# gutiKristian/VolumeRendering

Hardware: AMD Instinct MI355X
Metric: Gsamples/s (higher is better)
Workload: dtype f32

## Files before the change

volumerendering_amd/csrc/vr_p2.h:

```cpp
#pragma once
#include "vr_pw.h"

namespace VR_KNS {
using namespace vr;

#ifndef VR_P2_JUMP_MAX
#define VR_P2_JUMP_MAX 1024
#endif
constexpr int kP2JumpMax = VR_P2_JUMP_MAX;
#ifndef VR_P2_EXIT
#define VR_P2_EXIT 1
#endif
constexpr bool kP2Exit = VR_P2_EXIT != 0;
constexpr int kP2Threads = 768;
constexpr int kP2ThreadsUnlit = 1024;


struct P2Lds {
    unsigned off_x, off_y, off_z;
    int mx, my, mz;
    unsigned win_last;
    unsigned win_slabs;
    unsigned win_slots;
};

__device__ __forceinline__ uint2 lds_pair(unsigned byte_off)
{
    return *reinterpret_cast<const uint2*>(reinterpret_cast<const char*>(vr_lds_tf) + byte_off);
}

__device__ __forceinline__ void p2_fill_tables(const DevVolume& v, const P2Lds& L)
{
    char* lds = reinterpret_cast<char*>(vr_lds_tf);
    for (int e = (int)threadIdx.x; e <= v.nx; e += (int)blockDim.x) {
        const unsigned i0 = (unsigned)max(e - 1, 0), i1 = (unsigned)min(e, v.nx - 1);
        *reinterpret_cast<uint2*>(lds + L.off_x + (unsigned)e * 8u) =
            make_uint2((i0 >> kVbS) * kVbN + (i0 & kVbM), (i1 >> kVbS) * kVbN + (i1 & kVbM));
    }
    for (int e = (int)threadIdx.x; e <= v.ny; e += (int)blockDim.x) {
        const unsigned j0 = (unsigned)max(e - 1, 0), j1 = (unsigned)min(e, v.ny - 1);
        *reinterpret_cast<uint2*>(lds + L.off_y + (unsigned)e * 8u) =
            make_uint2((j0 >> kVbS) * v.brick_row + ((j0 & kVbM) << kVbS), (j1 >> kVbS) * v.brick_row + ((j1 & kVbM) << kVbS));
    }
    for (int e = (int)threadIdx.x; e <= v.nz; e += (int)blockDim.x) {
        const unsigned k0 = (unsigned)max(e - 1, 0), k1 = (unsigned)min(e, v.nz - 1);
        *reinterpret_cast<uint2*>(lds + L.off_z + (unsigned)e * 8u) =
            make_uint2((k0 >> kVbS) * v.brick_slab + ((k0 & kVbM) << (2u * kVbS)), (k1 >> kVbS) * v.brick_slab + ((k1 & kVbM) << (2u * kVbS)));
    }
}

struct P2Win {
    unsigned long long ptr;
    unsigned records;
    unsigned base;
};

template <int V>
__device__ __forceinline__ void p2_set_window(P2Win& win, const DevVolume& vol, unsigned first_slot, unsigned n_slots)
{
    const char* b = (V == V_BASIC) ? vol.a_base + (size_t)first_slot * 4u : reinterpret_cast<const char*>(vol.data) + (size_t)first_slot * 16u;
    win.ptr = (unsigned long long)reinterpret_cast<size_t>(b);
    win.records = n_slots;
    win.base = first_slot;
}
template <int V>
__device__ __forceinline__ __amdgpu_buffer_rsrc_t p2_descriptor(const P2Win& win)
{
    const unsigned lo = (unsigned)__builtin_amdgcn_readfirstlane((int)(unsigned)win.ptr), hi = (unsigned)__builtin_amdgcn_readfirstlane((int)(unsigned)(win.ptr >> 32));
    void* p = reinterpret_cast<void*>((size_t)(((unsigned long long)hi << 32) | lo));
    return __builtin_amdgcn_make_buffer_rsrc(p, V == V_BASIC ? 4 : 16, __builtin_amdgcn_readfirstlane((int)win.records), 0x00020000);
}
template <int V>
constexpr unsigned p2_window_slots() { return V == V_BASIC ? 0x3fffffffu : 0x0fffffffu; }

struct P2Addr {
    uint2 ex, ey, ez;
    float fx, fy, fz;
    int tz;
};
__device__ __forceinline__ P2Addr p2_address(const DevVolume& vol, const P2Lds& L, f3 q)
{
    P2Addr a;
    const float x = mad(q.x, (float)vol.nx, -0.5f), y = mad(q.y, (float)vol.ny, -0.5f), z = mad(q.z, (float)vol.nz, -0.5f);
    const float x0 = floorf(x), y0 = floorf(y), z0 = floorf(z);
    a.fx = x - x0;
    a.fy = y - y0;
    a.fz = z - z0;
    const int tx = min(max((int)x0, -1), L.mx), ty = min(max((int)y0, -1), L.my);
    a.tz = min(max((int)z0, -1), L.mz);
    a.ex = lds_pair(L.off_x + ((unsigned)(tx + 1) << 3));
    a.ey = lds_pair(L.off_y + ((unsigned)(ty + 1) << 3));
    a.ez = lds_pair(L.off_z + ((unsigned)(a.tz + 1) << 3));
    return a;
}
template <int V, bool MASKED, bool WIN, typename T>
__device__ __forceinline__ void p2_issue(const MarchParams& P0, const DevVolume& vol, const P2Lds& L, P2Win& win, int& n_in_w, const P2Addr& a, T (&X)[8],
                                         float& fx, float& fy, float& fz, unsigned long long keep, bool need, unsigned& dbyte, float& mrec)
{
    fx = a.fx;
    fy = a.fy;
    fz = a.fz;
    const uint2 ex = a.ex, ey = a.ey, ez = a.ez;
    const int tz = a.tz;
    unsigned az0 = ez.x, az1 = ez.y;
    if constexpr (WIN) {
        az0 -= win.base;
        az1 -= win.base;
        unsigned chk = need ? az0 : 0u;
        asm volatile("" : "+v"(chk));
        const unsigned long long out = vr_ballot(chk > L.win_last);
        if (out != 0) {
            const int kb = __builtin_amdgcn_readlane(max(tz, 0) >> kVbS, (int)__builtin_ctzll(out));
            const int span = (int)L.win_slabs - 2;
            const unsigned first = (unsigned)max(0, kb - span / 2) * vol.brick_slab, total = vol.brick_slab * (((unsigned)vol.nz + kVbM) >> kVbS);
            p2_set_window<V>(win, vol, first, min(total - first, L.win_slots));
            az0 = ez.x - win.base;
            az1 = ez.y - win.base;
            unsigned chk2 = need ? az0 : 0u;
            asm volatile("" : "+v"(chk2));
            if (vr_ballot(chk2 > L.win_last) != 0) n_in_w = 0;
        }
    }
    const unsigned r00 = ey.x + az0, r10 = ey.y + az0, r01 = ey.x + az1, r11 = ey.y + az1;
    unsigned o[8] = {r00 + ex.x, r00 + ex.y, r10 + ex.x, r10 + ex.y, r01 + ex.x, r01 + ex.y, r11 + ex.x, r11 + ex.y};
    if constexpr (MASKED) {
        static_assert(kBrickShift == (int)kVbS, "the skipping's bricks are the layout's bricks");
        const unsigned bid = (WIN ? o[0] + win.base : o[0]) >> (3u * kVbS);
        dbyte = dist_at(P0, (int)bid);
        if constexpr (V == V_VOLUME_MASK) mrec = brick_record(P0, (int)bid).y;
    }
    const __amdgpu_buffer_rsrc_t rsrc = p2_descriptor<V>(win);
    unsigned long long exec_saved = 0;
    if constexpr (MASKED) {
        asm volatile("" : "+v"(o[0]), "+v"(o[1]), "+v"(o[2]), "+v"(o[3]), "+v"(o[4]), "+v"(o[5]), "+v"(o[6]), "+v"(o[7]));
        __builtin_amdgcn_sched_barrier(0);
        asm volatile("s_mov_b64 %0, exec\n\ts_and_b64 exec, exec, %1" : "=&s"(exec_saved) : "s"(keep) : "scc");
    }
#pragma unroll
    for (int k = 0; k < 8; ++k) {
        if constexpr (V == V_BASIC) X[k] = __builtin_bit_cast(float, vr_struct_load_b32(rsrc, (int)o[k], 0, 0, 0));
        else X[k] = __builtin_bit_cast(vr_f4, vr_struct_load_b128(rsrc, (int)o[k], 0, 0, 0));
    }
    if constexpr (MASKED) {
        __builtin_amdgcn_sched_barrier(0);
        asm volatile("s_mov_b64 exec, %0" : : "s"(exec_saved));
        __builtin_amdgcn_sched_barrier(0);
    }
}

template <int V, bool MASKED, bool WIN, typename T>
__device__ __forceinline__ void p2_request(const MarchParams& P0, const DevVolume& vol, const P2Lds& L, P2Win& win, int& n_in_w, f3 q, T (&X)[8], float& fx,
                                           float& fy, float& fz, unsigned long long keep, bool need, unsigned& dbyte, float& mrec)
{
    const P2Addr a = p2_address(vol, L, q);
    p2_issue<V, MASKED, WIN>(P0, vol, L, win, n_in_w, a, X, fx, fy, fz, keep, need, dbyte, mrec);
}

__device__ __forceinline__ int wave_min_i32(int v)
{
    v = min(v, __builtin_amdgcn_update_dpp(v, v, 0xB1, 0xF, 0xF, false));
    v = min(v, __builtin_amdgcn_update_dpp(v, v, 0x4E, 0xF, 0xF, false));
    v = min(v, __builtin_amdgcn_update_dpp(v, v, 0x141, 0xF, 0xF, false));
    v = min(v, __builtin_amdgcn_update_dpp(v, v, 0x140, 0xF, 0xF, false));
    return min(min(__builtin_amdgcn_readlane(v, 0), __builtin_amdgcn_readlane(v, 16)), min(__builtin_amdgcn_readlane(v, 32), __builtin_amdgcn_readlane(v, 48)));
}

__device__ __forceinline__ bool p2_vote(const MarchParams& P0, bool sampled, float d, bool masked = false)
{
    int j = padded_texel(floorf(mad(d, (float)P0.tf[0].res_o, -0.5f)), P0.tf[0].res_o);
    j = (d - d == 0.0f) ? j : 0x7fffffff;
    j = masked ? 0x7fffffff : j;
    j = sampled ? j : (int)0x80000000;
    asm volatile("" : "+v"(j));
    return vr_ballot(j > P0.tf_zero_prefix) != 0;
}

template <int V, bool SKIP, bool WIN, bool BATCH>
__global__ __launch_bounds__(V == V_BASIC ? kP2ThreadsUnlit : kP2Threads) void march_p2_kernel(const MarchBatch B, const PwQueue Q)
{
    static_assert(V == V_LIGHT || V == V_BASIC || (V == V_VOLUME_MASK && SKIP), "lit / unlit shader; the three-volume composite with its brick records");
    constexpr int kSrc = (V == V_VOLUME_MASK) ? 2 : 0;
    constexpr bool kLit = V != V_BASIC;
    constexpr bool kExit = SKIP && kP2Exit;
    const MarchParams& P0 = B.frame[0];
    const DevVolume& vol = P0.vol[kSrc];
    P2Lds L;
    {
        const unsigned tf_bytes = (unsigned)(P0.tf[0].res_o + 2) * 16u;
        L.off_x = tf_bytes;
        L.off_y = L.off_x + (unsigned)(vol.nx + 1) * 8u;
        L.off_z = L.off_y + (unsigned)(vol.ny + 1) * 8u;
        L.mx = vol.nx - 1;
        L.my = vol.ny - 1;
        L.mz = vol.nz - 1;
        L.win_slots = WIN ? (Q.p2_window ? Q.p2_window : p2_window_slots<V>()) : 0u;
        L.win_slabs = WIN ? L.win_slots / vol.brick_slab : 0u;
        L.win_last = WIN ? (L.win_slabs - 2u) * vol.brick_slab + (kVbM << (2u * kVbS)) : 0u;
        const int n = P0.tf[0].res_o + 2;
        constexpr int kU = 6;
        for (int base = (int)threadIdx.x; base < n; base += kU * (int)blockDim.x) {
            float4 c[kU];
            float o[kU];
#pragma unroll
            for (int u = 0; u < kU; ++u) {
                const int j = min(base + u * (int)blockDim.x, n - 1);
                c[u] = P0.tf[0].color[j];
                o[u] = P0.tf[0].opacity[j];
            }
#pragma unroll
            for (int u = 0; u < kU; ++u) {
                const int j = base + u * (int)blockDim.x;
                if (j < n) vr_lds_tf[j] = make_float4(c[u].x, c[u].y, c[u].z, o[u]);
            }
        }
        p2_fill_tables(vol, L);
        __syncthreads();
    }
    const unsigned total_slots = vol.brick_slab * (((unsigned)vol.nz + kVbM) >> kVbS);
    const unsigned cls = blockIdx.x & 7u;
    const unsigned groups = (gridDim.x - cls + 7u) >> 3;
    const unsigned wib = (unsigned)__builtin_amdgcn_readfirstlane((int)(threadIdx.x >> 6));
    const unsigned wpb = blockDim.x >> 6;
    const unsigned nf = B.n_frames;
    const unsigned n_c = (Q.n_items >> 3) * nf;
    unsigned idx = wib * groups + (blockIdx.x >> 3);
    typedef typename std::conditional<kLit, vr_f4, float>::type Elem;
    const unsigned cur = cls;
    for (;;) {
        if (idx >= n_c) break;
        const unsigned item = batch_group(idx, nf), frame = idx - item * nf;
        const MarchParams& P = B.frame[(unsigned)__builtin_amdgcn_readfirstlane((int)frame)];
        const f3 light_pos = mk3(P.light_pos[0], P.light_pos[1], P.light_pos[2]), light_dif = mk3(P.light_dif[0], P.light_dif[1], P.light_dif[2]),
                 light_amb = mk3(P.light_amb[0], P.light_amb[1], P.light_amb[2]);
        const int steps_count = P.steps_count;
        const unsigned pos = (item << 3) | cur;
        int lb = (int)pos;
        if (P0.order != nullptr) lb = __builtin_amdgcn_readfirstlane((int)P0.order[pos]);
        const unsigned long long t_start = wall_clock64();
        const PixelSlot slot = map_pixel_at(P0, lb, 1, 0);
        const float bx0 = P.bmin[0], by0 = P.bmin[1], bz0 = P.bmin[2];
        const float bx1 = P.bmax[0], by1 = P.bmax[1], bz1 = P.bmax[2];
        float4 dst = make_float4(0.0f, 0.0f, 0.0f, 0.0f);
        unsigned blends = 0, covered = 0, fetched = 0;
#if VR_P2_DEBUG
        unsigned dbg_trips = 0, dbg_sampled = 0, dbg_shaded = 0, dbg_jumps = 0;
        unsigned long long dbg_wait_corners = 0, dbg_wait_bytes = 0, dbg_loop = 0;
        unsigned long long dbg_tail = 0;
        const unsigned long long dbg_pkt0 = __builtin_readcyclecounter();
#endif
        bool alive = false;
        f3 p = mk3(0.0f, 0.0f, 0.0f), w = p, step = p, wstep = p;
        int n_inside = 0;
        if (slot.active && slot.px >= P.rect[0] && slot.px <= P.rect[2] && slot.py >= P.rect[1] && slot.py <= P.rect[3]) {
            Ray ray = setup_ray(P, slot.px, slot.py);
            if (ray.hit) {
                covered = 1;
                f3 diff = mk3(ray.end.x - ray.start.x, ray.end.y - ray.start.y, ray.end.z - ray.start.z);
                f3 dir = normalize3s(diff);
                float ray_len = length3s(diff);
                if (P.fragment_mode == 1) {
                    dst = make_float4(fabsf(dir.x), fabsf(dir.y), fabsf(dir.z), 1.0f);
                } else if (P.fragment_mode == 2) {
                    dst = make_float4(ray.start.x, ray.start.y, ray.start.z, 1.0f);
                } else if (P.fragment_mode == 3) {
                    dst = make_float4(ray.end.x, ray.end.y, ray.end.z, 1.0f);
                } else if (P.fragment_mode == 4) {
                    dst = make_float4(0.5f * (ray.world0.x / 1.0f) + 0.5f, -0.5f * (ray.world0.y / 1.0f) + 0.5f, 0.0f, 1.0f);
                } else {
                    float step_size = P.step_size;
                    if constexpr (V == V_LIGHT) {
                        wstep = mk3(dir.x * (step_size * 1.0f), dir.y * (step_size * 1.0f), dir.z * (step_size * 0.5f));
                        wstep.z = wstep.z * (-1.0f);
                    }
                    if (P.toggle_varstep == 1) step_size = ray_len / (float)steps_count;
                    p = ray.start;
                    if (P.toggle_jitter == 1) {
                        float jt = jitter((float)slot.px + 0.5f, (float)slot.py + 0.5f);
                        p = mk3(p.x + (dir.x * step_size) * jt, p.y + (dir.y * step_size) * jt, p.z + (dir.z * step_size) * jt);
                    }
                    step = mk3(dir.x * step_size, dir.y * step_size, dir.z * step_size);
                    if constexpr (V == V_VOLUME_MASK) wstep = step;
                    w = ray.world0;
                    n_inside = steps_inside(p, step, bx0, by0, bz0, bx1, by1, bz1);
                    alive = steps_count > 0;
                }
            }
        }
        if (vr_ballot(alive) != 0) {
            Elem A[8], Bq[8];
#pragma unroll
            for (int k = 0; k < 8; ++k) {
                if constexpr (kLit) {
                    A[k] = vr_f4{0.0f, 0.0f, 0.0f, 0.0f};
                    Bq[k] = vr_f4{0.0f, 0.0f, 0.0f, 0.0f};
                } else {
                    A[k] = 0.0f;
                    Bq[k] = 0.0f;
                }
            }
            float afx = 0.0f, afy = 0.0f, afz = 0.0f, bfx = 0.0f, bfy = 0.0f, bfz = 0.0f;
            f3 pA = p, pB = p;
            int i = 0;
            int n_in_w = wave_min_i32(alive ? min(n_inside, steps_count) : 0x7fffffff);
            P2Win win;
            p2_set_window<V>(win, vol, 0u, WIN ? min(total_slots, L.win_slots) : total_slots);
            unsigned DA = 0, DB = 0;
            float MA = 0.0f, MB = 0.0f;
            float leap_c = 0.0f;
            int lim = 0;
            if constexpr (SKIP) {
                const float vmax = fmaxf(fmaxf(fabsf(step.x) * P0.bsx, fabsf(step.y) * P0.bsy), fabsf(step.z) * P0.bsz);
                leap_c = 0.999f / vmax;
                lim = min(n_inside, steps_count);
            }
            bool idle_a = false, idle_b = false;
            bool idle_ra = false, idle_rb = false;
            int mw = 0;
            auto one_step = [&](Elem (&X)[8], float& xfx, float& xfy, float& xfz, f3& pX, const f3& pY, int jump, bool idle_con, bool idle_rq, unsigned& DX,
                                float& MX) {
                const bool inb = alive;
                const bool sampled = SKIP ? (inb && !idle_con) : inb;
                f3 pN = mk3(pY.x + step.x, pY.y + step.y, pY.z + step.z);
                for (int k = 0; k < jump; ++k) pN = mk3(pN.x + step.x, pN.y + step.y, pN.z + step.z);
                const P2Addr ad = p2_address(vol, L, pN);
                v2f zw = v2f{0.0f, 0.0f}, gxy = zw;
                TfFetch tq;
                float4 mask = make_float4(0.0f, 0.0f, 0.0f, 0.0f);
                float rt = 0.0f;
                bool any_masked = false, masked = false;
                bool shaded = !SKIP || vr_ballot(!idle_con) != 0;
#if VR_P2_DEBUG
                if (shaded) ++dbg_sampled;
#endif
                if (shaded) {
#if VR_P2_DEBUG >= 2
                    const unsigned long long c0 = __builtin_readcyclecounter();
#endif
                    if constexpr (kLit) asm volatile("" : "+v"(X[0]), "+v"(X[1]), "+v"(X[2]), "+v"(X[3]), "+v"(X[4]), "+v"(X[5]), "+v"(X[6]), "+v"(X[7]));
                    else asm volatile("" : "+v"(X[0]), "+v"(X[1]), "+v"(X[2]), "+v"(X[3]), "+v"(X[4]), "+v"(X[5]), "+v"(X[6]), "+v"(X[7]));
#if VR_P2_DEBUG >= 2
                    dbg_wait_corners += __builtin_readcyclecounter() - c0;
#endif
                }
                if (!shaded) {
                } else if constexpr (kLit) {
                    Fetch4 q;
                    q.a = make_float4(X[0].x, X[0].y, X[0].z, X[0].w); q.b = make_float4(X[1].x, X[1].y, X[1].z, X[1].w);
                    q.d = make_float4(X[2].x, X[2].y, X[2].z, X[2].w); q.e = make_float4(X[3].x, X[3].y, X[3].z, X[3].w);
                    q.f = make_float4(X[4].x, X[4].y, X[4].z, X[4].w); q.g = make_float4(X[5].x, X[5].y, X[5].z, X[5].w);
                    q.h = make_float4(X[6].x, X[6].y, X[6].z, X[6].w); q.i = make_float4(X[7].x, X[7].y, X[7].z, X[7].w);
                    zw = interp_zw(q, xfx, xfy, xfz);
                    if constexpr (V == V_VOLUME_MASK) {
                        gxy = interp_xy(q, xfx, xfy, xfz);
                        asm volatile("" : "+v"(zw.x), "+v"(zw.y), "+v"(gxy.x), "+v"(gxy.y));
                        any_masked = vr_ballot(sampled && !(MX <= 0.0f)) != 0;
                        if (any_masked) {
                            mask = tex3_rgba<!WIN>(P0.vol[0], pX);
                            rt = tex3_a<!WIN>(P0.vol[1], pX);
                            asm volatile("" : "+v"(mask.x), "+v"(mask.y), "+v"(mask.z), "+v"(rt));
                            masked = mask.x > 0.0f || mask.y > 0.0f || mask.z > 0.0f;
                        }
                        shaded = p2_vote(P0, sampled, zw.y, masked);
                        if (shaded) tq = tf_fetch_lds(P0.tf[0], zw.y);
                    } else {
                        if constexpr (SKIP) shaded = p2_vote(P0, sampled, zw.y);
                        if (shaded) {
                            tq = tf_fetch_lds(P0.tf[0], zw.y);
                            gxy = interp_xy(q, xfx, xfy, xfz);
                        }
                    }
                } else {
                    Fetch1 q;
                    q.a = X[0]; q.b = X[1]; q.d = X[2]; q.e = X[3]; q.f = X[4]; q.g = X[5]; q.h = X[6]; q.i = X[7];
                    zw.y = interp_a(q, xfx, xfy, xfz);
                    if constexpr (SKIP) shaded = p2_vote(P0, sampled, zw.y);
                    if (shaded) tq = tf_fetch_lds(P0.tf[0], zw.y);
                }
                pX = pN;
                if constexpr (kLit) asm volatile("" : "+v"(zw.x), "+v"(zw.y), "+v"(gxy.x), "+v"(gxy.y));
                else asm volatile("" : "+v"(zw.y));
                __builtin_amdgcn_sched_barrier(0);
                const bool rq = alive && !(SKIP && idle_rq);
                p2_issue<V, SKIP, WIN>(P0, vol, L, win, n_in_w, ad, X, xfx, xfy, xfz, vr_ballot(rq), rq, DX, MX);
                __builtin_amdgcn_sched_barrier(0);
#if VR_P2_DEBUG
                if (shaded) ++dbg_shaded;
#endif
                if (sampled) {
                    if (shaded) {
                        if constexpr (V == V_LIGHT) {
                            shade_blend_packed<true>(light_pos, light_dif, light_amb, 2.5f, 0.5f, w, zw, gxy, tq, dst);
                        } else if constexpr (V == V_VOLUME_MASK) {
                            TfSample trt;
                            trt.rgb = mk3(0.0f, 0.0f, 0.0f);
                            trt.opacity = 0.0f;
                            if (any_masked) {
                                TfFetch rq = tf_fetch(P0.tf[1], rt);
                                tf_pin(rq);
                                trt = tf_finish(rq);
                            }
                            shade_blend_packed<true, true>(mk3(0.0f, -5.0f, 0.0f), mk3(0.96f, 0.76f, 0.67f), mk3(1.0f, 1.0f, 1.0f), 1.5f, 0.5f, w, zw, gxy, tq,
                                                           dst, masked, trt.rgb, trt.opacity);
                        } else {
                            const TfSample t = tf_finish(tq);
                            blend(t.rgb, t.opacity, dst);
                        }
                    }
                    ++fetched;
                }
                if (inb) ++blends;
                alive = alive && can_blend<V>(dst.w);
                if constexpr (kLit) w = mk3(w.x + wstep.x, w.y + wstep.y, w.z + wstep.z);
            };
            int k_last = 0x7fffffff;
            if constexpr (SKIP) {
                int k0, k1;
                steps_near_box(pA, step, P0.abox, steps_count, k0, k1);
                if constexpr (kExit) k_last = k1;
                int skipped = 0;
                while (i < n_in_w && vr_ballot(alive) != 0) {
                    const bool near = alive && i >= k0 && i <= k1;
                    int safe = kP2JumpMax;
                    if (vr_ballot(near) != 0) {
                        const unsigned d = dist_at(P0, brick_of<true>(P0, pA));
                        if (vr_ballot(near && d == 0u) != 0) break;
                        const int sf = 1 + max((int)fminf(((float)d - (1.0f + kBrickHalf)) * leap_c, (float)kP2JumpMax), 0);
                        safe = near ? sf : safe;
                    }
                    if (alive && i < k0) safe = min(safe, k0 - i);
                    safe = alive ? min(safe, lim - i) : kP2JumpMax;
                    const int sw = wave_min_i32(safe);
                    for (int k = 0; k < sw; ++k) pA = mk3(pA.x + step.x, pA.y + step.y, pA.z + step.z);
                    if (alive) blends += (unsigned)sw;
                    i += sw;
                    skipped += sw;
                }
                if constexpr (kLit) {
                    if (skipped != 0 && vr_ballot(alive && i <= k1) != 0)
                        for (int k = 0; k < skipped; ++k) w = mk3(w.x + wstep.x, w.y + wstep.y, w.z + wstep.z);
                }
                p = pA;
                pB = pA;
            }
            bool start = true;
#if VR_P2_DEBUG
            dbg_trips = dbg_sampled = dbg_shaded = dbg_jumps = 0;
            dbg_loop = __builtin_readcyclecounter();
#endif
            while (i + 2 <= n_in_w && vr_ballot(alive) != 0) {
                if constexpr (kExit) {
                    if (vr_ballot(alive && i <= k_last) == 0) break;
                }
                if (start) {
                    pB = mk3(pA.x + step.x, pA.y + step.y, pA.z + step.z);
                    p2_request<V, SKIP, WIN>(P0, vol, L, win, n_in_w, pA, A, afx, afy, afz, vr_ballot(alive), alive, DA, MA);
                    p2_request<V, SKIP, WIN>(P0, vol, L, win, n_in_w, pB, Bq, bfx, bfy, bfz, vr_ballot(alive), alive, DB, MB);
                    start = false;
                    if constexpr (WIN) {
                        if (n_in_w == 0) break;
                    }
                }
                mw = 0;
                if constexpr (SKIP) {
#if VR_P2_DEBUG >= 2
                    {
                        const unsigned long long c0 = __builtin_readcyclecounter();
                        asm volatile("" : "+v"(DA), "+v"(DB));
                        dbg_wait_bytes += __builtin_readcyclecounter() - c0;
                    }
#endif
                    unsigned da = alive ? DA : 255u, db = alive ? DB : 255u;
                    asm volatile("" : "+v"(da), "+v"(db));
                    idle_a = da >= 1u;
                    idle_b = db >= 1u;
                    int m = min((int)fminf(((float)db - (1.0f + kBrickHalf)) * leap_c, (float)kP2JumpMax), lim - (i + 1) - 1);
                    m = alive ? m : kP2JumpMax;
                    if (vr_ballot(m < 1) == 0) mw = min(wave_min_i32(m), kP2JumpMax);
                    idle_ra = m >= mw + 1;
                    idle_rb = m >= mw + 2;
                }
#if VR_P2_DEBUG
                ++dbg_trips;
                if (mw > 0) ++dbg_jumps;
#endif
                one_step(A, afx, afy, afz, pA, pB, mw, idle_a, idle_ra, DA, MA);
                one_step(Bq, bfx, bfy, bfz, pB, pA, 0, idle_b, idle_rb, DB, MB);
                if (mw > 0) {
                    if constexpr (kLit) {
                        for (int k = 0; k < mw; ++k) w = mk3(w.x + wstep.x, w.y + wstep.y, w.z + wstep.z);
                    }
                    if (alive) blends += (unsigned)mw;
                }
                i += 2 + mw;
            }
#if VR_P2_DEBUG
            dbg_loop = __builtin_readcyclecounter() - dbg_loop;
            dbg_tail = __builtin_readcyclecounter();
#endif
            if (!start) p = pA;
            if constexpr (kExit) {
                if (i < n_in_w && vr_ballot(alive) != 0 && vr_ballot(alive && i <= k_last) == 0) {
                    const int sw = n_in_w - i;
                    for (int k = 0; k < sw; ++k) p = mk3(p.x + step.x, p.y + step.y, p.z + step.z);
                    if (alive) blends += (unsigned)sw;
                    i += sw;
                }
            }
            for (; i < steps_count && vr_ballot(alive) != 0; ++i) {
                if (alive) {
                    bool inb = true;
                    if (i >= n_inside) inb = p.x >= bx0 && p.x <= bx1 && p.y >= by0 && p.y <= by1 && p.z >= bz0 && p.z <= bz1;
                    if (inb) {
                        bool sampled = true;
                        if constexpr (SKIP) sampled = i <= k_last && dist_at(P0, brick_of<true>(P0, p)) == 0u;
                        if (sampled) {
                            sample_and_blend<V, !WIN, SKIP, true>(P, p, w, dst, mk3(0.0f, 0.0f, 0.0f), 0.0f);
                            ++fetched;
                        }
                        ++blends;
                        if (!can_blend<V>(dst.w)) alive = false;
                    } else {
                        const bool gone = (step.x >= 0.0f && p.x > bx1) || (step.x <= 0.0f && p.x < bx0) || (step.y >= 0.0f && p.y > by1) ||
                                          (step.y <= 0.0f && p.y < by0) || (step.z >= 0.0f && p.z > bz1) || (step.z <= 0.0f && p.z < bz0);
                        if (gone) alive = false;
                    }
                }
                p = mk3(p.x + step.x, p.y + step.y, p.z + step.z);
                if constexpr (kLit) w = mk3(w.x + wstep.x, w.y + wstep.y, w.z + wstep.z);
            }
        }
#if VR_P2_DEBUG
        if (dbg_tail) dbg_tail = __builtin_readcyclecounter() - dbg_tail;
#endif
        if (slot.active || (P0.packed && slot.in_launch)) P.out[slot.out_index] = dst;
        store_wave_counts(P, lb, blends, covered, fetched, t_start);
#if VR_P2_DEBUG
        if ((threadIdx.x & 63) == 0)
            P.block_counts[(size_t)lb * kBlockRecord + 2] = (unsigned long long)(dbg_trips & 0xfffu) | ((unsigned long long)(dbg_sampled & 0xfffu) << 12) |
                                                           ((unsigned long long)(dbg_shaded & 0xfffu) << 24) | ((unsigned long long)(dbg_jumps & 0xfffu) << 36);
#if VR_P2_DEBUG >= 2
        if ((threadIdx.x & 63) == 0)
#if VR_P2_DEBUG >= 3
            P.block_counts[(size_t)lb * kBlockRecord + 1] = ((dbg_tail >> 6) & 0xfffffull) | ((((__builtin_readcyclecounter() - dbg_pkt0) >> 6) & 0xfffffull) << 20) |
                                                           (((dbg_loop >> 6) & 0xffffffull) << 40);
#else
            P.block_counts[(size_t)lb * kBlockRecord + 1] = ((dbg_wait_corners >> 6) & 0xfffffull) | (((dbg_wait_bytes >> 6) & 0xfffffull) << 20) |
                                                           (((dbg_loop >> 6) & 0xffffffull) << 40);
#endif
#endif
#endif
        unsigned r = 0;
        if ((threadIdx.x & 63u) == 0) r = atomicAdd(Q.heads + cur * kPwHeadStride, 1u);
        idx = groups * wpb + (unsigned)__builtin_amdgcn_readfirstlane((int)r);
    }
}

}
```

Before: 373.0.

## Probe several distance-field bricks per empty-space approach iteration

The empty-space skipping loop now reads the brick distance field at a window of up to four consecutive ray steps per iteration instead of one. It then computes the furthest safe reach across the window, which cuts the number of wave-wide ballot and min-reduction rounds before the ray reaches occupied space. In exchange each iteration issues several dependent brick and distance lookups, adds register pressure, and may fetch distances past where a single probe would already have stopped. Debug-only cycle counters for the approach phase are added as well.

```diff
diff --git a/volumerendering_amd/csrc/vr_approach.h b/volumerendering_amd/csrc/vr_approach.h
--- /dev/null
+++ b/volumerendering_amd/csrc/vr_approach.h
@@ -0,0 +1,30 @@
+#pragma once
+#include "vr_choice.h"
+
+namespace vr {
+
+constexpr float kApproachBias = 1.0f + 0.5f / (float)kBrickCells;
+
+constexpr int approach_bound(unsigned d, float leap_c, int jump_max)
+{
+    const float b = ((float)d - kApproachBias) * leap_c;
+    return b >= (float)jump_max ? jump_max : (b > 0.0f ? (int)b : 0);
+}
+
+template <int K>
+constexpr int approach_run(const unsigned (&d)[K], const bool (&near)[K], float leap_c, int to_lim, int to_k0, int jump_max, bool& stop)
+{
+    int reach = to_k0 > 0 ? to_k0 : 0;
+    int zero = K;
+    for (int k = K - 1; k >= 0; --k) {
+        const bool seen = k < to_lim;
+        const int by_byte = k + 1 + approach_bound(d[k], leap_c, jump_max);
+        const int own = near[k] ? by_byte : (k < to_k0 ? 0 : k + jump_max);
+        reach = (seen && own > reach) ? own : reach;
+        zero = (seen && near[k] && d[k] == 0u) ? k : zero;
+    }
+    stop = zero < K;
+    return stop ? zero : (reach < to_lim ? reach : to_lim);
+}
+
+}
diff --git a/volumerendering_amd/csrc/vr_p2.h b/volumerendering_amd/csrc/vr_p2.h
--- a/volumerendering_amd/csrc/vr_p2.h
+++ b/volumerendering_amd/csrc/vr_p2.h
@@ -1,4 +1,5 @@
 #pragma once
+#include "vr_approach.h"
 #include "vr_pw.h"
 
 namespace VR_KNS {
@@ -8,6 +9,13 @@
 #define VR_P2_JUMP_MAX 1024
 #endif
 constexpr int kP2JumpMax = VR_P2_JUMP_MAX;
+#ifndef VR_P2_WINDOW
+#define VR_P2_WINDOW 4
+#endif
+constexpr int kP2Window = VR_P2_WINDOW;
+static_assert(kP2Window >= 1 && kP2Window <= 16 && kApproachBias == 1.0f + kBrickHalf, "the approach's window; the one-byte rule's bias");
+template <int V, bool WIN>
+constexpr int p2_approach_window() { return (V == V_VOLUME_MASK || WIN) ? 1 : kP2Window; }
 #ifndef VR_P2_EXIT
 #define VR_P2_EXIT 1
 #endif
@@ -246,6 +254,8 @@
         unsigned dbg_trips = 0, dbg_sampled = 0, dbg_shaded = 0, dbg_jumps = 0;
         unsigned long long dbg_wait_corners = 0, dbg_wait_bytes = 0, dbg_loop = 0;
         unsigned long long dbg_tail = 0;
+        unsigned dbg_app_it = 0;
+        unsigned long long dbg_app = 0;
         const unsigned long long dbg_pkt0 = __builtin_readcyclecounter();
 #endif
         bool alive = false;
@@ -418,23 +428,44 @@
                 steps_near_box(pA, step, P0.abox, steps_count, k0, k1);
                 if constexpr (kExit) k_last = k1;
                 int skipped = 0;
+                constexpr int kWin = p2_approach_window<V, WIN>();
+#if VR_P2_DEBUG
+                dbg_app = __builtin_readcyclecounter();
+#endif
                 while (i < n_in_w && vr_ballot(alive) != 0) {
-                    const bool near = alive && i >= k0 && i <= k1;
-                    int safe = kP2JumpMax;
-                    if (vr_ballot(near) != 0) {
-                        const unsigned d = dist_at(P0, brick_of<true>(P0, pA));
-                        if (vr_ballot(near && d == 0u) != 0) break;
-                        const int sf = 1 + max((int)fminf(((float)d - (1.0f + kBrickHalf)) * leap_c, (float)kP2JumpMax), 0);
-                        safe = near ? sf : safe;
-                    }
-                    if (alive && i < k0) safe = min(safe, k0 - i);
-                    safe = alive ? min(safe, lim - i) : kP2JumpMax;
-                    const int sw = wave_min_i32(safe);
+#if VR_P2_DEBUG
+                    ++dbg_app_it;
+#endif
+                    const int to_lim = lim - i, to_k0 = k0 - i;
+                    const int lo = max(to_k0, 0), hi = alive ? min(min(k1 - i, to_lim - 1), kWin - 1) : -1;
+                    unsigned d[kWin];
+                    bool near[kWin];
+#pragma unroll
+                    for (int k = 0; k < kWin; ++k) {
+                        near[k] = k >= lo && k <= hi;
+                        d[k] = 1u;
+                    }
+                    if (vr_ballot(lo <= hi) != 0) {
+                        f3 q = pA;
+#pragma unroll
+                        for (int k = 0; k < kWin; ++k) {
+                            const int bid = brick_of<true>(P0, q);
+                            d[k] = dist_at(P0, near[k] ? bid : 0);
+                            q = mk3(q.x + step.x, q.y + step.y, q.z + step.z);
+                        }
+                    }
+                    bool stop;
+                    const int run = approach_run<kWin>(d, near, leap_c, to_lim, to_k0, kP2JumpMax, stop);
+                    const int sw = wave_min_i32(alive ? run : 0x7fffffff);
                     for (int k = 0; k < sw; ++k) pA = mk3(pA.x + step.x, pA.y + step.y, pA.z + step.z);
                     if (alive) blends += (unsigned)sw;
                     i += sw;
                     skipped += sw;
-                }
+                    if (vr_ballot(alive && stop && run == sw) != 0) break;
+                }
+#if VR_P2_DEBUG
+                dbg_app = __builtin_readcyclecounter() - dbg_app;
+#endif
                 if constexpr (kLit) {
                     if (skipped != 0 && vr_ballot(alive && i <= k1) != 0)
                         for (int k = 0; k < skipped; ++k) w = mk3(w.x + wstep.x, w.y + wstep.y, w.z + wstep.z);
@@ -537,10 +568,14 @@
 #if VR_P2_DEBUG
         if ((threadIdx.x & 63) == 0)
             P.block_counts[(size_t)lb * kBlockRecord + 2] = (unsigned long long)(dbg_trips & 0xfffu) | ((unsigned long long)(dbg_sampled & 0xfffu) << 12) |
-                                                           ((unsigned long long)(dbg_shaded & 0xfffu) << 24) | ((unsigned long long)(dbg_jumps & 0xfffu) << 36);
+                                                           ((unsigned long long)(dbg_shaded & 0xfffu) << 24) | ((unsigned long long)(dbg_jumps & 0xfffu) << 36) |
+                                                           ((unsigned long long)min(dbg_app_it, 0xffffu) << 48);
 #if VR_P2_DEBUG >= 2
         if ((threadIdx.x & 63) == 0)
-#if VR_P2_DEBUG >= 3
+#if VR_P2_DEBUG >= 4
+            P.block_counts[(size_t)lb * kBlockRecord + 1] = ((dbg_tail >> 6) & 0xfffffull) | (((dbg_app >> 6) & 0xfffffull) << 20) |
+                                                           ((((__builtin_readcyclecounter() - dbg_pkt0) >> 6) & 0xffffffull) << 40);
+#elif VR_P2_DEBUG >= 3
             P.block_counts[(size_t)lb * kBlockRecord + 1] = ((dbg_tail >> 6) & 0xfffffull) | ((((__builtin_readcyclecounter() - dbg_pkt0) >> 6) & 0xfffffull) << 20) |
                                                            (((dbg_loop >> 6) & 0xffffffull) << 40);
 #else
```

Result: no change. 376.0, median of 6 (+0.8%).
